# openai/tiktoken

Measured on AMD Instinct MI355X. Metric: GB/s text encoded (o200k_base-shaped vocab, 1 GiB corpus per GPU), bit-exact vs CoreBPE restatement, higher is better.
Workload: dtype u8; 1 GPU; o200k_shaped encode_ordinary_batch, 1024 MiB synthetic web-text per GPU (tkc_generate mix=1, seed 0x5EED0003), 318404 docs on rank 0, inputs resident in HBM, packed u32 output; encoding=o200k_shaped, pat_str_runs_on=hand-written scanners, bytes_per_gpu=1073741824, docs_rank0=318404, rccl_ranks=0, devices_visible=1, pieces_rank0=162498410, parallelism=doc-sharded x1

## Files before the change

tiktoken_amd/csrc/tk_common.h:

```cpp
#pragma once
#include <stdint.h>

#if defined(__HIPCC__)
#include <hip/hip_runtime.h>
#define TK_HD __host__ __device__ __forceinline__
#else
#define TK_HD inline
#endif

#define TK_RANK_MAX 0xFFFFFFFFu
#define TK_TILE 3840

enum : int {
    TK_DBG_SCANNERS = 4,
    TK_DBG_STARTS_ONLY = 8,
    TK_DBG_VERBOSE = 64,
    TK_DBG_KEEP_LONG = 0x80,
    TK_DBG_NO_MT = 256,
    TK_DBG_COLLIDE = 512,
    TK_DBG_ONE_MERGE = 1024,
    TK_DBG_NO_SMALL = 2048,
    TK_DBG_GENERIC = 0x100000,
    TK_DBG_NO_MID_CUT = 0x200000,
    TK_DBG_MERGE_PER_BIN = 0x800000,
    TK_DBG_NO_BUDGET = 0x20000000,
    TK_DBG_MAY_GIVE_UP = 0x8000000,
    TK_DBG_SECOND = 0x10000000,
    TK_DBG_HARD_ONLY = 0x40000000,
    TK_DBG_INTERNAL = TK_DBG_MAY_GIVE_UP | TK_DBG_SECOND | TK_DBG_HARD_ONLY,
};
constexpr int TK_DBG_USER[] = {TK_DBG_SCANNERS, TK_DBG_STARTS_ONLY, TK_DBG_VERBOSE, TK_DBG_KEEP_LONG, TK_DBG_NO_MT, TK_DBG_COLLIDE, TK_DBG_ONE_MERGE,
                               TK_DBG_NO_SMALL, TK_DBG_GENERIC, TK_DBG_NO_MID_CUT, TK_DBG_MERGE_PER_BIN, TK_DBG_NO_BUDGET};
constexpr bool tk_dbg_user_bits_disjoint() {
    int seen = TK_DBG_INTERNAL;
    for (int b : TK_DBG_USER) {
        if ((b & (b - 1)) != 0 || (seen & b) != 0) return false;
        seen |= b;
    }
    return true;
}
static_assert(tk_dbg_user_bits_disjoint(), "a debug bit a user sets is shared");

enum { TK_PAT_R50K = 0, TK_PAT_CL100K = 1, TK_PAT_O200K = 2 };

enum {
    TK_C_CONT = 0,
    TK_C_NL = 1,
    TK_C_SP = 2,
    TK_C_WSO = 3,
    TK_C_LU = 4,
    TK_C_LL = 5,
    TK_C_LC = 6,
    TK_C_MK = 7,
    TK_C_NU = 8,
    TK_C_AP = 9,
    TK_C_SL = 10,
    TK_C_OT = 11,
    TK_C_END = 12,
    TK_C_SPEC = 13,
};
#define TK_F_HARD 0x80u
#define TK_CB(c) (1u << (c))
#define TK_M_WS (TK_CB(TK_C_NL) | TK_CB(TK_C_SP) | TK_CB(TK_C_WSO))
#define TK_M_L (TK_CB(TK_C_LU) | TK_CB(TK_C_LL) | TK_CB(TK_C_LC))
#define TK_M_OTHER (TK_CB(TK_C_MK) | TK_CB(TK_C_AP) | TK_CB(TK_C_SL) | TK_CB(TK_C_OT))
#define TK_M_WORD (TK_M_L | TK_CB(TK_C_MK))
#define TK_M_UPPERISH (TK_CB(TK_C_LU) | TK_CB(TK_C_LC) | TK_CB(TK_C_MK))
#define TK_M_LOWERISH (TK_CB(TK_C_LL) | TK_CB(TK_C_LC) | TK_CB(TK_C_MK))

struct TkPieceSlot {
    uint64_t key;
    uint32_t rank;
    uint32_t len;
};
struct TkShortSlot {
    uint32_t key;
    uint32_t val;
};
#define TK_SHORT_EMPTY 0xFFFFFFFFu
#define TK_SHORT_RANK_MASK 0x3FFFFFFFu
#define TK_SHORT_MAX_RANK 0x3FFFFFFEu
#define TK_XL_MIN 9u
#define TK_XL_MAX 23u
struct alignas(16) TkXlSlot {
    uint64_t w0, w1, w2;
    uint32_t rank;
    uint32_t pad;
};
struct TkPairSlot {
    uint64_t key;
    uint32_t rank;
    uint32_t pad;
};
#define TK_EMPTY_KEY 0xFFFFFFFFFFFFFFFFull

struct TkPat {
    uint32_t w0;
    uint32_t c1;
    uint32_t c2[2];
    TK_HD constexpr int fam() const { return (int)(w0 & 3u); }
    TK_HD constexpr bool ci() const { return (w0 >> 2) & 1u; }
    TK_HD constexpr uint32_t suffix() const { return (w0 >> 3) & 3u; }
    TK_HD constexpr bool generic() const { return (w0 >> 5) & 1u; }
    TK_HD constexpr bool ws_dollar() const { return (w0 >> 6) & 1u; }
    TK_HD constexpr bool nl_rule() const { return (w0 >> 7) & 1u; }
    TK_HD constexpr uint32_t digits() const { return (w0 >> 8) & 0xFFu; }
    TK_HD constexpr uint32_t n2() const { return (w0 >> 16) & 7u; }
    TK_HD constexpr uint32_t two(uint32_t i) const { return (c2[i >> 1] >> (16u * (i & 1u))) & 0xFFFFu; }
    TK_HD constexpr uint32_t suffix_mask() const { return ((suffix() & 1u) ? TK_CB(TK_C_NL) : 0u) | ((suffix() & 2u) ? TK_CB(TK_C_SL) : 0u); }
    TK_HD constexpr bool same_as(const TkPat& o) const { return ((w0 ^ o.w0) & ~32u) == 0u && c1 == o.c1 && c2[0] == o.c2[0] && c2[1] == o.c2[1]; }
};
#define TK_PAT_GENERIC 3
TK_HD constexpr TkPat tk_stock_pat(int fam) {
    return TkPat{(uint32_t)fam | (fam != TK_PAT_R50K ? 4u : 0u) | (fam == TK_PAT_CL100K ? 8u : (fam == TK_PAT_O200K ? 24u : 0u)) |
                     (fam != TK_PAT_O200K ? 64u : 0u) | (fam != TK_PAT_R50K ? 128u : 0u) | (fam != TK_PAT_R50K ? (3u << 8) : 0u) | (3u << 16),
                 (1u << ('s' - 'a')) | (1u << ('t' - 'a')) | (1u << ('m' - 'a')) | (1u << ('d' - 'a')),
                 {((uint32_t)'l' << 8 | 'l') | (((uint32_t)'v' << 8 | 'e') << 16), ((uint32_t)'r' << 8 | 'e')}};
}

struct TkTables {
    const uint8_t* uc_stage1;
    const uint8_t* uc_stage2;
    const uint8_t* uc_bmp;
    const uint32_t* byte_tab;
    const TkShortSlot* short_tab;
    uint32_t short_mask, short_shift;
    const TkPieceSlot* mid_tab;
    uint32_t mid_mask, mid_shift;
    const TkPieceSlot* piece;
    const uint32_t* piece_off;
    uint64_t piece_mask;
    uint32_t max_token_len;
    const uint8_t* tok_bytes;
    const TkPairSlot* pair;
    const uint64_t* pair8;
    uint64_t pair_mask;
    const uint32_t* pair2;
    const uint32_t* byte_rank;
    const uint8_t* spec_bytes;
    const uint32_t* spec_off;
    const uint32_t* spec_id;
    const uint32_t* spec_head;
    uint32_t n_spec;
    uint32_t spec_first[8];
    uint32_t spec_fb;
    uint32_t n_spec_fb;
    uint32_t spec_second[8];
    int pattern;
    TkPat pat;
    uint16_t cert[16];
    const struct TkXlSlot* xl;
    uint32_t xl_mask;
    const uint32_t* xfilter;
};
#define TK_XFILTER_BITS (1u << 20)
TK_HD uint32_t tk_xfilter_bit(uint64_t ident_hash) { return (uint32_t)(ident_hash >> 32) & (TK_XFILTER_BITS - 1u); }

TK_HD uint64_t tk_mix64(uint64_t x) {
    x ^= x >> 32;
    x *= 0xD6E8FEB86659FD93ull;
    x ^= x >> 32;
    x *= 0xD6E8FEB86659FD93ull;
    x ^= x >> 32;
    return x;
}

TK_HD uint64_t tk_piece_slot_hash(uint64_t key, uint32_t len) {
    uint32_t x = (uint32_t)key * 0x9E3779B1u;
    x ^= x >> 15;
    x += (uint32_t)(key >> 32) * 0x85EBCA77u + len * 0xC2B2AE3Du;
    x ^= x >> 13;
    x *= 0x27D4EB2Fu;
    x ^= x >> 16;
    return x;
}
TK_HD uint32_t tk_short_slot(uint32_t key, uint32_t shift) { return (key * 0x9E3779B1u) >> shift; }
TK_HD uint32_t tk_mid_slot(uint64_t key, uint32_t shift) {
    uint32_t x = (uint32_t)key * 0x9E3779B1u + (uint32_t)(key >> 32) * 0x85EBCA77u;
    x ^= x >> 15;
    return (x * 0xC2B2AE3Du) >> shift;
}
TK_HD uint64_t tk_pair_slot_hash(uint64_t key) {
    uint32_t x = (uint32_t)key * 0x9E3779B1u + (uint32_t)(key >> 32) * 0x85EBCA77u;
    x ^= x >> 15;
    x *= 0x2C1B3C6Du;
    x ^= x >> 12;
    x *= 0x297A2D39u;
    x ^= x >> 15;
    return x;
}

TK_HD uint64_t tk_keep_bytes(uint64_t x, int r) {
    const uint32_t t4 = 4u * (8u - (uint32_t)(r < 0 ? 0 : (r > 8 ? 8 : r)));
    return (x << t4) << t4;
}
template <class Ld8>
TK_HD void tk_ident(Ld8&& ld8, uint32_t len, uint32_t where, uint64_t& w0, uint64_t& w1, uint64_t& w2) {
    const bool exact = len <= TK_XL_MAX;
    const uint64_t x0 = ld8(0u), x1 = ld8(exact ? 8u : len - 8u);
    w0 = tk_keep_bytes(x0, (int)len);
    w1 = exact ? tk_keep_bytes(x1, (int)len - 8) : x1;
    w2 = (1ull << 63) | ((uint64_t)len << 32) | where;
    if (exact) w2 = (tk_keep_bytes(ld8(16u), (int)len - 16) >> 8) | ((uint64_t)len << 56);
}
TK_HD uint64_t tk_ident_hash(uint64_t w0, uint64_t w1, uint64_t w2, bool exact) {
    const uint32_t a = (uint32_t)w0, b = (uint32_t)(w0 >> 32), c = (uint32_t)w1, d = (uint32_t)(w1 >> 32);
    const uint32_t e = exact ? (uint32_t)w2 : 0u, f = (uint32_t)(w2 >> 32);
    uint32_t h1 = a * 0x9E3779B1u + b * 0x85EBCA77u + c * 0xC2B2AE3Du + d * 0x27D4EB2Fu + e * 0x165667B1u + f * 0xD3A2646Du;
    h1 ^= h1 >> 15;
    h1 *= 0x2C1B3C6Du;
    h1 ^= h1 >> 12;
    uint32_t h2 = (a ^ 0x5BD1E995u) * 0x7FEB352Du + (b + d) * 0x846CA68Bu + (c ^ f) * 0xFD7046C5u + (e + ((a >> 19) | (a << 13))) * 0xB55A4F09u;
    h2 ^= h2 >> 13;
    h2 *= 0x9E3779B1u;
    h2 ^= h2 >> 16;
    return ((uint64_t)h2 << 32) | h1;
}

TK_HD uint64_t tk_hash_step(uint64_t h, uint64_t w) {
    uint64_t x = (h ^ w) * 0x9FB21C651E98DF25ull;
    x ^= x >> 29;
    return x + 0x9E3779B97F4A7C15ull;
}
#define TK_HASH_SEED 0x243F6A8885A308D3ull
#define TK_KEY_SAMPLED 32u
#define TK_PAIR8_ID_BITS 21
#define TK_PAIR8_MAX_ID ((1u << TK_PAIR8_ID_BITS) - 2u)
```

tiktoken_amd/csrc/tk_device.h:

```cpp
#pragma once
#include "tk_common.h"

TK_HD uint32_t tk_class_of_cp(const TkTables& T, uint32_t cp) {
    if (cp > 0x10FFFFu) return TK_C_OT;
    return T.uc_stage2[(uint32_t)T.uc_stage1[cp >> 8] * 256u + (cp & 255u)];
}

TK_HD uint32_t tk_classify_text(const TkTables& T, const uint8_t* __restrict__ text, uint64_t pos, uint64_t n) {
    uint32_t b = text[pos];
    if (b < 0x80u) return tk_class_of_cp(T, b);
    if ((b & 0xC0u) == 0x80u) return TK_C_CONT;
    uint32_t len = b >= 0xF0u ? 4u : (b >= 0xE0u ? 3u : 2u);
    if (pos + len > n) return TK_C_OT;
    uint32_t cp;
    if (len == 2u)
        cp = ((b & 0x1Fu) << 6) | (text[pos + 1] & 0x3Fu);
    else if (len == 3u)
        cp = ((b & 0x0Fu) << 12) | ((uint32_t)(text[pos + 1] & 0x3Fu) << 6) | (text[pos + 2] & 0x3Fu);
    else
        cp = ((b & 0x07u) << 18) | ((uint32_t)(text[pos + 1] & 0x3Fu) << 12) |
             ((uint32_t)(text[pos + 2] & 0x3Fu) << 6) | (text[pos + 3] & 0x3Fu);
    return tk_class_of_cp(T, cp);
}

// ... 480 lines not shown
            if (pat.generic() && !sx) break;
            sx &= sx - 1;
        }
        e = sx ? tk_ctz64(sx) : r;
        return e > TK_WIN_SAFE ? 0 : e;
    }
    uint32_t s = 0;
    bool s_ok = true;
    if (c == TK_C_SP && !nxt_end) s = k1;
    if (pat.fam() == TK_PAT_R50K) {
        int kind = -1;
        uint64_t b0 = 0;
        if ((w.get(TKB_L) >> s) & 1ull) { kind = TKB_L; b0 = w.get(TKB_L); }
        else if ((w.get(TKB_NU) >> s) & 1ull) { kind = TKB_NU; b0 = w.get(TKB_NU); }
        else if ((w.get(TKB_OTH) >> s) & 1ull) { kind = TKB_OTH; b0 = w.get(TKB_OTH); }
        if (kind >= 0) {
            uint32_t r = tk_runx(b0, stop, x, kind, s);
            return r == TK_UNRES ? 0 : s + r;
        }
        s_ok = false;
    } else if ((w.get(TKB_OTH) >> s) & 1ull) {
        uint32_t r = tk_runx(w.get(TKB_OTH), stop, x, TKB_OTH, s);
        if (r == TK_UNRES) return 0;
        const uint32_t e1 = s + r;
        uint32_t r2 = (pat.fam() == TK_PAT_O200K || pat.generic()) ? tk_runx(w.get(TKB_NLSL), stop, x, TKB_NLSL, e1) : tk_runx(w.get(TKB_NL), stop, x, TKB_NL, e1);
        return r2 == TK_UNRES ? 0 : e1 + r2;
    } else {
        s_ok = false;
    }
    (void)s_ok;
    {
        uint32_t q = tk_runx(w.get(TKB_WS), stop, x, TKB_WS, 0);
        if (q == TK_UNRES) return 0;
        if (q <= TK_WIN_SAFE) {
            uint64_t rng = tk_below(q);
            bool at_end = (stop >> q) & 1ull;
            uint64_t nlr = w.get(TKB_NL) & rng, st = w.start & rng;
            if (pat.ws_dollar() && at_end) return q;
            if (pat.nl_rule() && nlr) return 64u - tk_clz64(nlr);
            if (at_end) return q;
            if (tk_popc64(st) >= 2u) return 63u - tk_clz64(st);
            return q;
        }
        if (q + 1u > x.limit()) return 0;
        const bool at_end = tk_bitx(w.stop, x, TKB_HARD, q);
        if (pat.ws_dollar() && at_end) return q;
        if (pat.nl_rule()) {
            int ln = tk_last_setx(w.get(TKB_NL), x, TKB_NL, 0, q);
            if (ln >= 0) return (uint32_t)ln + 1u;
        }
        if (at_end) return q;
        return (uint32_t)tk_last_setx(w.start, x, TKB_START, 0, q);
    }
}

#define TK_WIN32_SAFE 26u
#if defined(__HIP_DEVICE_COMPILE__)
TK_HD uint32_t tk_w32_ctz(uint32_t v) { return v ? (uint32_t)(__ffs((int)v) - 1) : 32u; }
TK_HD uint32_t tk_w32_clz(uint32_t v) { return v ? (uint32_t)__clz((int)v) : 32u; }
TK_HD uint32_t tk_w32_popc(uint32_t v) { return (uint32_t)__popc(v); }
#else
TK_HD uint32_t tk_w32_ctz(uint32_t v) { return v ? (uint32_t)__builtin_ctz(v) : 32u; }
TK_HD uint32_t tk_w32_clz(uint32_t v) { return v ? (uint32_t)__builtin_clz(v) : 32u; }
TK_HD uint32_t tk_w32_popc(uint32_t v) { return (uint32_t)__builtin_popcount(v); }
#endif
TK_HD uint32_t tk_below32(uint32_t b) { return b >= 32u ? ~0u : ((1u << b) - 1u); }
TK_HD uint32_t tk_run32(uint32_t bits, uint32_t stop, uint32_t from) {
    return tk_w32_ctz(~((bits & ~stop) >> from));
}

template <class W32, class A>
TK_HD uint32_t tk_piece_len_bits32(const W32& w, A& a, uint64_t p, uint32_t c, TkPat pat) {
    const uint32_t stop = w.stop;
    const uint32_t k1 = 1u + tk_w32_ctz((w.start | stop) >> 1);
    if (k1 > 4u || c == TK_C_SPEC) return 0;
    const bool nxt_end = (stop >> k1) & 1u;
    uint32_t e = 0;
    if (pat.fam() == TK_PAT_O200K) {
        uint32_t ks = 64;
        if ((TK_M_WORD >> c) & 1u) ks = 0;
        else if (c != TK_C_NL && c != TK_C_NU && !nxt_end && (((w.get(TKB_UP) | w.get(TKB_LOW)) >> k1) & 1u)) ks = k1;
        if (ks != 64u) {
            const uint32_t re = ks + tk_run32(w.get(TKB_UP), stop, ks);
            if (re > TK_WIN32_SAFE) return 0;
            const uint32_t te = re + tk_run32(w.get(TKB_LOW), stop, re);
            if (te > TK_WIN32_SAFE) return 0;
            if (te > re) {
                e = te;
            } else {
                const uint32_t xx = w.get(TKB_CAS) & ~stop & tk_below32(re) & ~tk_below32(ks);
                e = xx ? 32u - tk_w32_clz(xx) : re;
            }
            if (!((stop >> e) & 1u) && a.byte(p + e) == '\'') e += tk_contraction_bits(w, a, p, e, pat);
            return e;
        }
    } else if (pat.fam() == TK_PAT_CL100K) {
        if (c == TK_C_AP) {
            const uint32_t k = tk_contraction_bits(w, a, p, 0, pat);
            if (k) return k;
        }
        if ((TK_M_L >> c) & 1u) {
            const uint32_t r = tk_run32(w.get(TKB_L), stop, 0);
            return r > TK_WIN32_SAFE ? 0 : r;
        }
        if (c != TK_C_NL && c != TK_C_NU && !nxt_end && ((w.get(TKB_L) >> k1) & 1u)) {
            const uint32_t r = k1 + tk_run32(w.get(TKB_L), stop, k1);
            return r > TK_WIN32_SAFE ? 0 : r;
        }
    } else {
        if (c == TK_C_AP) {
            const uint32_t k = tk_contraction_bits(w, a, p, 0, pat);
            if (k) return k;
        }
    }
    if (pat.fam() != TK_PAT_R50K && c == TK_C_NU) {
        const uint32_t r = tk_run32(w.get(TKB_NU), stop, 0);
        uint32_t sx = pat.digits() ? (w.start & tk_below32(r)) : 0u;
        for (uint32_t i = 0; i < pat.digits(); ++i) {
            if (pat.generic() && !sx) break;
            sx &= sx - 1;
        }
        e = sx ? tk_w32_ctz(sx) : r;
        return e > TK_WIN32_SAFE ? 0 : e;
    }
    uint32_t s = 0;
    if (c == TK_C_SP && !nxt_end) s = k1;
    if (pat.fam() == TK_PAT_R50K) {
        int kind = -1;
        if ((w.get(TKB_L) >> s) & 1u) kind = TKB_L;
        else if ((w.get(TKB_NU) >> s) & 1u) kind = TKB_NU;
        else if ((w.get(TKB_OTH) >> s) & 1u) kind = TKB_OTH;
        if (kind >= 0) {
            const uint32_t r = s + tk_run32(w.get(kind), stop, s);
            return r > TK_WIN32_SAFE ? 0 : r;
        }
    } else if ((w.get(TKB_OTH) >> s) & 1u) {
        const uint32_t e1 = s + tk_run32(w.get(TKB_OTH), stop, s);
        if (e1 > TK_WIN32_SAFE) return 0;
        const uint32_t e2 = e1 + tk_run32((pat.fam() == TK_PAT_O200K || pat.generic()) ? w.get(TKB_NLSL) : w.get(TKB_NL), stop, e1);
        return e2 > TK_WIN32_SAFE ? 0 : e2;
    }
    const uint32_t q = tk_run32(w.get(TKB_WS), stop, 0);
    if (q > TK_WIN32_SAFE) return 0;
    const uint32_t rng = tk_below32(q);
    const bool at_end = (stop >> q) & 1u;
    const uint32_t nlr = w.get(TKB_NL) & rng, st = w.start & rng;
    if (pat.ws_dollar() && at_end) return q;
    if (pat.nl_rule() && nlr) return 32u - tk_w32_clz(nlr);
    if (at_end) return q;
    if (tk_w32_popc(st) >= 2u) return 31u - tk_w32_clz(st);
    return q;
}

TK_HD uint32_t tk_probe_short_from(const TkTables& T, uint32_t key, uint32_t len, uint32_t i, TkShortSlot s) {
    for (;;) {
        if (s.key == key && (s.val >> 30) == len - 1u && s.val != TK_SHORT_EMPTY) return s.val & TK_SHORT_RANK_MASK;
        if (s.val == TK_SHORT_EMPTY) return TK_RANK_MAX;
        i = (i + 1u) & T.short_mask;
        s = T.short_tab[i];
    }
}
TK_HD uint32_t tk_probe_short(const TkTables& T, uint32_t key, uint32_t len) {
    const uint32_t i = tk_short_slot(key, T.short_shift);
    return tk_probe_short_from(T, key, len, i, T.short_tab[i]);
}
TK_HD uint32_t tk_probe_mid_from(const TkTables& T, uint64_t key, uint32_t len, uint32_t i, TkPieceSlot s) {
    for (;;) {
        if (s.key == key && s.len == len) return s.rank;
        if (s.len == 0u) return TK_RANK_MAX;
        i = (i + 1u) & T.mid_mask;
        s = T.mid_tab[i];
    }
}
TK_HD uint32_t tk_probe_mid(const TkTables& T, uint64_t key, uint32_t len) {
    const uint32_t i = tk_mid_slot(key, T.mid_shift);
    return tk_probe_mid_from(T, key, len, i, T.mid_tab[i]);
}
template <class Verify>
TK_HD uint32_t tk_probe_piece_from(const TkTables& T, uint64_t key, uint32_t len, uint64_t i, TkPieceSlot s, Verify verify) {
    for (;;) {
        if (s.key == TK_EMPTY_KEY && s.len == 0u) return TK_RANK_MAX;
        if (s.key == key && s.len == len && verify(T.piece_off[i])) return s.rank;
        i = (i + 1) & T.piece_mask;
        s = T.piece[i];
    }
}
template <class Verify>
TK_HD uint32_t tk_probe_piece(const TkTables& T, uint64_t key, uint32_t len, Verify verify) {
    const uint64_t i = tk_piece_slot_hash(key, len) & T.piece_mask;
    return tk_probe_piece_from(T, key, len, i, T.piece[i], verify);
}

TK_HD uint32_t tk_probe_xl_from(const TkTables& T, uint64_t w0, uint64_t w1, uint64_t w2, uint32_t i, TkXlSlot s) {
    for (;;) {
        if (s.rank == TK_RANK_MAX) return TK_RANK_MAX;
        if (s.w0 == w0 && s.w1 == w1 && s.w2 == w2) return s.rank;
        i = (i + 1u) & T.xl_mask;
        s = T.xl[i];
    }
}
TK_HD uint32_t tk_probe_xl(const TkTables& T, uint64_t w0, uint64_t w1, uint64_t w2) {
    const uint32_t i = (uint32_t)tk_ident_hash(w0, w1, w2, true) & T.xl_mask;
    return tk_probe_xl_from(T, w0, w1, w2, i, T.xl[i]);
}

TK_HD uint32_t tk_probe_pair(const TkTables& T, uint32_t a, uint32_t b) {
    if (T.pair8) {
        const uint64_t key = ((uint64_t)a << TK_PAIR8_ID_BITS) | b;
        uint64_t bk = tk_pair_slot_hash(key) & T.pair_mask;
        for (;;) {
            const uint64_t* p = T.pair8 + bk * 4;
#if defined(__HIP_DEVICE_COMPILE__)
            const ulonglong2 v0 = *(const ulonglong2*)p, v1 = *(const ulonglong2*)(p + 2);
            const uint64_t s0 = v0.x, s1 = v0.y, s2 = v1.x, s3 = v1.y;
#else
            const uint64_t s0 = p[0], s1 = p[1], s2 = p[2], s3 = p[3];
#endif
            if ((s0 >> 22) == key) return (uint32_t)(s0 & 0x3FFFFFu);
            if ((s1 >> 22) == key) return (uint32_t)(s1 & 0x3FFFFFu);
            if ((s2 >> 22) == key) return (uint32_t)(s2 & 0x3FFFFFu);
            if ((s3 >> 22) == key) return (uint32_t)(s3 & 0x3FFFFFu);
            if (s3 == TK_EMPTY_KEY) return TK_RANK_MAX;
            bk = (bk + 1) & T.pair_mask;
        }
    }
    uint64_t key = ((uint64_t)a << 32) | b;
    uint64_t i = tk_pair_slot_hash(key) & T.pair_mask;
    for (;;) {
        TkPairSlot s = T.pair[i];
        if (s.key == key) return s.rank;
        if (s.key == TK_EMPTY_KEY) return TK_RANK_MAX;
        i = (i + 1) & T.pair_mask;
    }
}

TK_HD uint64_t tk_load8(const uint8_t* __restrict__ text, uint64_t pos) {
    uintptr_t a = (uintptr_t)(text + pos);
    const uint64_t* w = (const uint64_t*)(a & ~(uintptr_t)7);
    uint32_t sh = (uint32_t)(a & 7u) * 8u;
    uint64_t lo = w[0];
    if (sh == 0) return lo;
    uint64_t hi = w[1];
    return (lo >> sh) | (hi << (64u - sh));
}

TK_HD uint64_t tk_mask_low_bytes(uint64_t w, uint32_t nbytes) {
    return nbytes >= 8u ? w : (w & ((1ull << (nbytes * 8u)) - 1ull));
}

TK_HD uint64_t tk_key_of_text(const uint8_t* __restrict__ text, uint64_t pos, uint32_t len) {
    if (len <= 8u) return tk_mask_low_bytes(tk_load8(text, pos), len);
    if (len > TK_KEY_SAMPLED) {
        uint64_t h = TK_HASH_SEED ^ ((uint64_t)len << 32);
        h = tk_hash_step(h, tk_load8(text, pos));
        h = tk_hash_step(h, tk_load8(text, pos + 8u));
        h = tk_hash_step(h, tk_load8(text, pos + len - 16u));
        h = tk_hash_step(h, tk_load8(text, pos + len - 8u));
        return h == TK_EMPTY_KEY ? 0 : h;
    }
    uint64_t h = TK_HASH_SEED;
    uint32_t i = 0;
    for (; i + 8u <= len; i += 8u) h = tk_hash_step(h, tk_load8(text, pos + i));
    if (i < len) h = tk_hash_step(h, tk_mask_low_bytes(tk_load8(text, pos + i), len - i));
    if (h == TK_EMPTY_KEY) h = 0;
    return h;
}

TK_HD bool tk_equal_bytes(const uint8_t* text, uint64_t pos, const uint8_t* blob, uint32_t off, uint32_t len) {
    uint32_t i = 0;
    for (; i + 8u <= len; i += 8u)
        if (tk_load8(text, pos + i) != tk_load8(blob, (uint64_t)off + i)) return false;
    if (i < len) {
        uint32_t r = len - i;
        if (tk_mask_low_bytes(tk_load8(text, pos + i), r) != tk_mask_low_bytes(tk_load8(blob, (uint64_t)off + i), r)) return false;
    }
    return true;
}

TK_HD uint32_t tk_lookup_text_piece(const TkTables& T, const uint8_t* __restrict__ text, uint64_t pos, uint32_t len) {
    if (len <= 8u) {
        const uint64_t key = tk_mask_low_bytes(tk_load8(text, pos), len);
        if (len <= 4u && T.short_tab) return tk_probe_short(T, (uint32_t)key, len);
        return tk_probe_mid(T, key, len);
    }
    if (len > T.max_token_len) return TK_RANK_MAX;
    uint64_t key = tk_key_of_text(text, pos, len);
    return tk_probe_piece(T, key, len, [&](uint32_t off) { return tk_equal_bytes(text, pos, T.tok_bytes, off, len); });
}

#if defined(__HIP_DEVICE_COMPILE__)
TK_HD int tk_ffs32(uint32_t v) { return __ffs((int)v); }
TK_HD int tk_clz32(uint32_t v) { return __clz((int)v); }
TK_HD int tk_popc32(uint32_t v) { return __popc(v); }
#else
TK_HD int tk_ffs32(uint32_t v) { return __builtin_ffs((int)v); }
TK_HD int tk_clz32(uint32_t v) { return v ? __builtin_clz(v) : 32; }
TK_HD int tk_popc32(uint32_t v) { return __builtin_popcount(v); }
#endif

struct TkMask128 {
    uint64_t lo, hi;
    TK_HD void clear(uint32_t k) {
        if (k < 64u) lo &= ~(1ull << k);
        else hi &= ~(1ull << (k - 64u));
    }
    TK_HD bool test(uint32_t k) const { return k < 64u ? (lo >> k) & 1ull : (hi >> (k - 64u)) & 1ull; }
    TK_HD uint32_t next_after(uint32_t k) const {
        if (k < 63u) {
            uint64_t l = lo & ~((2ull << k) - 1ull);
            if (l) return tk_ctz64(l);
        }
        uint64_t h = hi;
        if (k >= 127u) h = 0;
        else if (k >= 64u) h &= ~((2ull << (k - 64u)) - 1ull);
        if (h) return 64u + tk_ctz64(h);
        return 128u;
    }
    TK_HD int prev_before(uint32_t k) const {
        uint64_t h = k > 64u ? hi & ((1ull << (k - 64u)) - 1ull) : 0ull;
        if (h) return 127 - (int)tk_clz64(h);
        uint64_t l = k >= 64u ? lo : lo & ((1ull << k) - 1ull);
        if (l) return 63 - (int)tk_clz64(l);
        return -1;
    }
};

template <int STRIDE>
TK_HD uint32_t tk_lane_merge(const TkTables& T, const uint8_t* __restrict__ text, uint64_t s, uint32_t n, uint32_t* id, uint32_t* rk,
                             uint32_t* __restrict__ out) {
    uint32_t pb = text[s];
    for (uint32_t k = 0; k < n; ++k) {
        uint32_t nb = k + 1 < n ? text[s + k + 1] : 0u;
        id[k * STRIDE] = T.byte_rank[pb];
        rk[k * STRIDE] = k + 1 < n ? T.pair2[(pb << 8) | nb] : TK_RANK_MAX;
        pb = nb;
    }
    TkMask128 alive;
    alive.lo = n >= 64u ? ~0ull : ((1ull << n) - 1ull);
    alive.hi = n > 64u ? (n >= 128u ? ~0ull : ((1ull << (n - 64u)) - 1ull)) : 0ull;
    for (;;) {
        uint32_t best = TK_RANK_MAX, bi = 0;
        for (uint32_t k = 0; k + 1 < n; ++k) {
            uint32_t r = rk[k * STRIDE];
            if (r < best) {
                best = r;
                bi = k;
            }
        }
        if (best == TK_RANK_MAX) break;
        const uint32_t j = alive.next_after(bi);
        alive.clear(j);
        id[bi * STRIDE] = best;
        rk[j * STRIDE] = TK_RANK_MAX;
        const uint32_t nn = alive.next_after(bi);
        const int pp = alive.prev_before(bi);
        uint32_t r_i = TK_RANK_MAX, r_p = TK_RANK_MAX;
// ... 11 lines not shown
```

tiktoken_amd/csrc/tk_tables.cpp:

```cpp
#include "tk_tables.h"

#include <stdio.h>
#include <stdlib.h>
#include <string.h>

#include <algorithm>
#include <array>
#include <chrono>
#include <numeric>
#include <thread>

int tk_pattern_id(const char* pat_str) {
    TkPat p;
    TkRxCompiled rx;
    if (!tk_compile_pattern(pat_str, &p, nullptr, &rx).empty()) return -1;
    return rx.empty() ? p.fam() : 3;
}

TkPat tk_nosplit_pat() { return TkPat{(uint32_t)TK_PAT_R50K | 32u, 0u, {0u, 0u}}; }

std::string tk_compile_pattern(const char* pat_str, TkPat* pat, uint16_t* cert, TkRxCompiled* rx) {
    const char* dbg = getenv("TIKTOKEN_AMD_DEBUG");
    const bool force_generic = dbg && (atoi(dbg) & TK_DBG_GENERIC);
    const std::string perr = force_generic ? std::string("generic engine forced by TIKTOKEN_AMD_DEBUG") : tk_parse_pattern(pat_str, pat, cert);
    if (perr.empty()) return "";
    const std::string rerr = tk_rx_compile(pat_str, rx);
    if (!rerr.empty()) {
        rx->ins.clear();
        return "pat_str is not supported: " + rerr + " [and it is not one of the hand-written scanner families: " + perr + "]";
    }
    *pat = tk_nosplit_pat();
    if (cert) memset(cert, 0, 16 * sizeof(uint16_t));
    return "";
}

uint64_t tk_key_of_bytes(const uint8_t* p, uint32_t len) {
    if (len <= 8) {
        uint64_t k = 0;
        memcpy(&k, p, len);
        return k;
    }
    if (len > TK_KEY_SAMPLED) {
        uint64_t h = TK_HASH_SEED ^ ((uint64_t)len << 32);
        for (uint32_t o : {0u, 8u, len - 16u, len - 8u}) {
            uint64_t w;
            memcpy(&w, p + o, 8);
            h = tk_hash_step(h, w);
        }
        return h == TK_EMPTY_KEY ? 0 : h;
    }
    uint64_t h = TK_HASH_SEED;
    uint32_t i = 0;
    for (; i + 8 <= len; i += 8) {
        uint64_t w;
        memcpy(&w, p + i, 8);
        h = tk_hash_step(h, w);
    }
    if (i < len) {
        uint64_t w = 0;
        memcpy(&w, p + i, len - i);
        h = tk_hash_step(h, w);
    }
    if (h == TK_EMPTY_KEY) h = 0;
    return h;
}

uint32_t TkHostTables::lookup_piece(const uint8_t* p, uint32_t len) const {
    if (len == 0) return TK_RANK_MAX;
    if (len <= 8) {
        uint64_t key = 0;
        memcpy(&key, p, len);
        if (len <= 4 && !short_tab.empty()) {
            uint32_t i = tk_short_slot((uint32_t)key, short_shift);
            for (;;) {
                const TkShortSlot& s = short_tab[i];
                if (s.val == TK_SHORT_EMPTY) return TK_RANK_MAX;
                if (s.key == (uint32_t)key && (s.val >> 30) == len - 1) return s.val & TK_SHORT_RANK_MASK;
                i = (i + 1) & short_mask;
            }
        }
        if (mid_tab.empty()) return TK_RANK_MAX;
        uint32_t i = tk_mid_slot(key, mid_shift);
        for (;;) {
            const TkPieceSlot& s = mid_tab[i];
            if (s.len == 0) return TK_RANK_MAX;
            if (s.key == key && s.len == len) return s.rank;
            i = (i + 1) & mid_mask;
        }
    }
    if (piece.empty()) return TK_RANK_MAX;
    uint64_t key = tk_key_of_bytes(p, len);
    uint64_t i = tk_piece_slot_hash(key, len) & piece_mask;
    for (;;) {
        const TkPieceSlot& s = piece[i];
        if (s.key == TK_EMPTY_KEY && s.len == 0) return TK_RANK_MAX;
        if (s.key == key && s.len == len) {
            if (memcmp(tok_bytes.data() + piece_off[i], p, len) == 0) return s.rank;
        }
        i = (i + 1) & piece_mask;
    }
}

uint32_t TkHostTables::lookup_pair(uint32_t a, uint32_t b) const {
    if (!pair8.empty()) {
        const uint64_t key = ((uint64_t)a << TK_PAIR8_ID_BITS) | b;
        uint64_t bk = tk_pair_slot_hash(key) & pair_mask;
        for (;;) {
            for (int j = 0; j < 4; ++j) {
                uint64_t s = pair8[bk * 4 + j];
                if ((s >> 22) == key) return (uint32_t)(s & 0x3FFFFFu);
                if (s == TK_EMPTY_KEY) return TK_RANK_MAX;
            }
            bk = (bk + 1) & pair_mask;
        }
    }
    uint64_t key = ((uint64_t)a << 32) | b;
    uint64_t i = tk_pair_slot_hash(key) & pair_mask;
    for (;;) {
        const TkPairSlot& s = pair[i];
        if (s.key == TK_EMPTY_KEY) return TK_RANK_MAX;
        if (s.key == key) return s.rank;
        i = (i + 1) & pair_mask;
    }
}

std::string tk_build_tables(const uint8_t* ranks_blob, const uint64_t* ranks_off, const uint32_t* ranks_ids,
                            uint64_t n_ranks, const uint8_t* spec_blob, const uint64_t* spec_off,
                            const uint32_t* spec_ids, uint64_t n_spec, const char* pat_str, TkHostTables* out) {
    TkHostTables& T = *out;
    const bool timing = getenv("TIKTOKEN_AMD_TIMING") != nullptr;
    auto t_prev = std::chrono::steady_clock::now();
    auto lap = [&](const char* what) {
        const auto now = std::chrono::steady_clock::now();
        if (timing) fprintf(stderr, "tk_build_tables: %-28s %7.1f ms\n", what, std::chrono::duration<double, std::milli>(now - t_prev).count());
        t_prev = now;
    };
    {
        const std::string perr = tk_compile_pattern(pat_str, &T.pat, T.cert, &T.rx);
        if (!perr.empty()) return perr;
        T.pattern = T.pat.fam();
    }
    lap("pattern");
    if (n_ranks == 0) return "mergeable_ranks is empty";
    if (ranks_off[n_ranks] >= 0xFFFFFFFFull) return "vocabulary byte blob too large";
    T.n_ranks = n_ranks;
    T.tok_bytes.assign(ranks_blob, ranks_blob + ranks_off[n_ranks]);
    T.tok_bytes.resize(T.tok_bytes.size() + 16, 0);

    uint32_t max_rank = 0;
    uint64_t n_short = 0, n_mid = 0, n_long = 0, n_xl = 0;
    for (uint64_t k = 0; k < n_ranks; ++k) {
        max_rank = std::max(max_rank, ranks_ids[k] == TK_RANK_MAX ? 0u : ranks_ids[k]);
        const uint64_t len = ranks_off[k + 1] - ranks_off[k];
        (len <= 4 ? n_short : (len <= 8 ? n_mid : n_long)) += 1;
        if (len >= TK_XL_MIN && len <= TK_XL_MAX) ++n_xl;
    }
    for (uint64_t k = 0; k < n_spec; ++k) max_rank = std::max(max_rank, spec_ids[k]);
    if (max_rank >= 0x7FFFFFFFu)
        return "token ids of 2^31 - 1 and above are not supported (the per-piece result word keeps its top bit for pieces that are not a "
               "single token, and one value for text that yields no token)";
    const bool use_short = max_rank <= TK_SHORT_MAX_RANK;
    if (!use_short) {
        n_mid += n_short;
        n_short = 0;
    }
    auto pow2_for = [](uint64_t items, uint32_t* mask, uint32_t* shift) {
        uint32_t bits = 6;
        while ((1ull << bits) < 2 * items + 2) ++bits;
        *mask = (uint32_t)((1ull << bits) - 1);
        *shift = 32 - bits;
        return (uint64_t)1 << bits;
    };
    if (use_short) T.short_tab.assign(pow2_for(n_short, &T.short_mask, &T.short_shift), TkShortSlot{0xFFFFFFFFu, TK_SHORT_EMPTY});
    T.mid_tab.assign(pow2_for(n_mid, &T.mid_mask, &T.mid_shift), TkPieceSlot{TK_EMPTY_KEY, TK_RANK_MAX, 0});
    uint64_t cap = 64;
    while (cap < 2 * n_long + 2) cap <<= 1;
    T.piece_mask = cap - 1;
    T.piece.assign(cap, TkPieceSlot{TK_EMPTY_KEY, TK_RANK_MAX, 0});
    T.piece_off.assign(cap, 0);
    {
        uint64_t xcap = 64;
        while (2 * xcap < 5 * n_xl + 2) xcap <<= 1;
        T.xl_mask = (uint32_t)(xcap - 1);
        T.xl.assign(xcap, TkXlSlot{~0ull, ~0ull, ~0ull, TK_RANK_MAX, 0u});
        T.xfilter.assign(TK_XFILTER_BITS / 32, 0u);
    }
    for (int b = 0; b < 256; ++b) T.byte_rank[b] = TK_RANK_MAX;
    T.pair2.assign(65536, TK_RANK_MAX);
    {
        uint32_t mr = 0;
        for (uint64_t k = 0; k < n_ranks; ++k) mr = std::max(mr, ranks_ids[k] == TK_RANK_MAX ? 0u : ranks_ids[k]);
        T.max_rank = mr;
        T.dec_is_dense = (uint64_t)mr < 4 * n_ranks + 65536;
        if (T.dec_is_dense) T.dec_dense.assign((size_t)mr + 1, std::make_pair(0u, 0u));
        else T.dec_sparse.reserve(n_ranks * 2);
    }
    uint64_t pr_short = 0, pr_mid = 0, pr_long = 0, pr_xl = 0;
    for (uint64_t k = 0; k < n_ranks; ++k) {
        uint64_t o = ranks_off[k], len64 = ranks_off[k + 1] - o;
        if (len64 == 0) return "mergeable_ranks contains an empty key";
        uint32_t len = (uint32_t)len64, rank = ranks_ids[k];
        if (rank == TK_RANK_MAX) return "rank 0xFFFFFFFF is reserved (Rank::MAX sentinel, src/lib.rs:53)";
        const uint8_t* p = ranks_blob + o;
        if (T.lookup_piece(p, len) != TK_RANK_MAX) return "duplicate key in mergeable_ranks";
        bool fresh;
        if (T.dec_is_dense) {
            fresh = T.dec_dense[rank].second == 0;
            T.dec_dense[rank] = std::make_pair((uint32_t)o, len);
        } else {
            fresh = T.dec_sparse.emplace(rank, std::make_pair((uint32_t)o, len)).second;
        }
        if (!fresh)
            return "Encoder and decoder must be of equal length. Maybe you had duplicate token indices in your "
                   "encoder?";
        if (len <= 8) {
            uint64_t key = 0;
            memcpy(&key, p, len);
            if (len <= 4 && use_short) {
                uint32_t i = tk_short_slot((uint32_t)key, T.short_shift);
                ++pr_short;
                while (T.short_tab[i].val != TK_SHORT_EMPTY) {
                    i = (i + 1) & T.short_mask;
                    ++pr_short;
                }
                T.short_tab[i] = TkShortSlot{(uint32_t)key, rank | ((len - 1) << 30)};
            } else {
                uint32_t i = tk_mid_slot(key, T.mid_shift);
                ++pr_mid;
                while (T.mid_tab[i].len != 0) {
                    i = (i + 1) & T.mid_mask;
                    ++pr_mid;
                }
                T.mid_tab[i] = TkPieceSlot{key, rank, len};
            }
        } else {
            uint64_t key = tk_key_of_bytes(p, len);
            uint64_t i = tk_piece_slot_hash(key, len) & T.piece_mask;
            ++pr_long;
            while (!(T.piece[i].key == TK_EMPTY_KEY && T.piece[i].len == 0)) {
                i = (i + 1) & T.piece_mask;
                ++pr_long;
            }
            T.piece[i] = TkPieceSlot{key, rank, len};
            T.piece_off[i] = (uint32_t)o;
            uint64_t w0, w1, w2;
            tk_ident([&](uint32_t at) {
                uint64_t w = 0;
                memcpy(&w, p + at, at < len ? std::min<uint32_t>(8u, len - at) : 0u);
                return w;
            }, len, 0u, w0, w1, w2);
            if (len > TK_XL_MAX) {
                uint64_t hh = tk_ident_hash(w0, w1, w2, false);
                if (hh == TK_EMPTY_KEY) hh = 0;
                const uint32_t bit = tk_xfilter_bit(hh);
                T.xfilter[bit >> 5] |= 1u << (bit & 31u);
            }
            if (len >= TK_XL_MIN && len <= TK_XL_MAX) {
                uint32_t j = (uint32_t)tk_ident_hash(w0, w1, w2, true) & T.xl_mask;
                ++pr_xl;
                while (T.xl[j].rank != TK_RANK_MAX) {
                    j = (j + 1) & T.xl_mask;
                    ++pr_xl;
                }
                T.xl[j] = TkXlSlot{w0, w1, w2, rank, 0u};
            }
        }
        if (len == 1) T.byte_rank[p[0]] = rank;
        if (len == 2) T.pair2[((uint32_t)p[0] << 8) | p[1]] = rank;
        if (len > T.max_token_len) T.max_token_len = len;
    }
    T.probes_short = n_short ? (double)pr_short / (double)n_short : 0;
    T.probes_mid = n_mid ? (double)pr_mid / (double)n_mid : 0;
    T.probes_long = n_long ? (double)pr_long / (double)n_long : 0;
    T.probes_xl = n_xl ? (double)pr_xl / (double)n_xl : 0;
    for (int b = 0; b < 256; ++b)
        if (T.byte_rank[b] == TK_RANK_MAX)
            return "every single byte must be a key of mergeable_ranks (byte_pair_encode indexes ranks[piece] for "
                   "1-byte pieces, src/lib.rs:201-203)";

    lap("piece tables + decoder");
    std::vector<TkPairSlot> entries;
    {
        unsigned nth = std::thread::hardware_concurrency();
        nth = nth == 0 ? 1 : (nth > 32 ? 32 : nth);
        if (const char* e = getenv("TIKTOKEN_AMD_BUILD_THREADS")) nth = (unsigned)std::max(1, atoi(e));
        if (n_ranks < 4096) nth = 1;
        const uint64_t nblocks = (n_ranks + 255) / 256;
        std::vector<std::vector<TkPairSlot>> part(nblocks);
        auto work = [&](unsigned t) {
            for (uint64_t b = t; b < nblocks; b += nth) {
                std::vector<TkPairSlot>& e = part[b];
                for (uint64_t k = b * 256; k < b * 256 + 256 && k < n_ranks; ++k) {
                    uint64_t o = ranks_off[k];
                    uint32_t len = (uint32_t)(ranks_off[k + 1] - o), rank = ranks_ids[k];
                    const uint8_t* p = ranks_blob + o;
                    for (uint32_t s = 1; s < len; ++s) {
                        uint32_t a = T.lookup_piece(p, s);
                        if (a == TK_RANK_MAX) continue;
                        uint32_t b2 = T.lookup_piece(p + s, len - s);
                        if (b2 == TK_RANK_MAX) continue;
                        e.push_back(TkPairSlot{((uint64_t)a << 32) | b2, rank, 0});
                    }
                }
            }
        };
        std::vector<std::thread> th;
        for (unsigned t = 1; t < nth; ++t) th.emplace_back(work, t);
        work(0);
        for (auto& x : th) x.join();
        size_t tot = 0;
        for (auto& e : part) tot += e.size();
        entries.reserve(tot);
        for (auto& e : part) entries.insert(entries.end(), e.begin(), e.end());
    }
    T.n_pairs = entries.size();
    lap("pair entries");

    uint32_t max_id = 0;
    for (uint64_t k = 0; k < n_ranks; ++k) max_id = std::max(max_id, ranks_ids[k]);
    if (max_id <= TK_PAIR8_MAX_ID) {
        uint64_t nb = 16;
        while ((double)nb * 4 * 0.5 < (double)entries.size() + 1) nb <<= 1;
        T.pair_mask = nb - 1;
        T.pair8.assign(nb * 4, TK_EMPTY_KEY);
        for (const TkPairSlot& e : entries) {
            const uint64_t key = ((e.key >> 32) << TK_PAIR8_ID_BITS) | (e.key & 0xFFFFFFFFull);
            uint64_t bk = tk_pair_slot_hash(key) & T.pair_mask;
            for (;;) {
                int j = 0;
                while (j < 4 && T.pair8[bk * 4 + j] != TK_EMPTY_KEY) ++j;
                if (j < 4) {
                    T.pair8[bk * 4 + j] = (key << 22) | e.rank;
                    break;
                }
                bk = (bk + 1) & T.pair_mask;
            }
        }
    } else {
        cap = 64;
        while ((double)cap * 0.4 < (double)entries.size() + 1) cap <<= 1;
        T.pair_mask = cap - 1;
        T.pair.assign(cap, TkPairSlot{TK_EMPTY_KEY, TK_RANK_MAX, 0});
        for (const TkPairSlot& e : entries) {
            uint64_t i = tk_pair_slot_hash(e.key) & T.pair_mask;
            while (T.pair[i].key != TK_EMPTY_KEY) i = (i + 1) & T.pair_mask;
            T.pair[i] = e;
        }
    }

    lap("pair table");
    std::vector<uint64_t> order(n_spec);
    std::iota(order.begin(), order.end(), 0);
    auto sbytes = [&](uint64_t k) { return std::string((const char*)spec_blob + spec_off[k], spec_off[k + 1] - spec_off[k]); };
    std::sort(order.begin(), order.end(), [&](uint64_t a, uint64_t b) { return sbytes(a) < sbytes(b); });
    memset(T.spec_first, 0, sizeof T.spec_first);
    T.spec_off.push_back(0);
    for (uint64_t idx : order) {
        std::string s = sbytes(idx);
        if (s.empty()) return "empty special token";
        T.spec_decoder.emplace(spec_ids[idx], std::make_pair((uint32_t)T.spec_bytes.size(), (uint32_t)s.size()));
        T.spec_bytes.insert(T.spec_bytes.end(), s.begin(), s.end());
        T.spec_off.push_back((uint32_t)T.spec_bytes.size());
        T.spec_id.push_back(spec_ids[idx]);
        unsigned char f = (unsigned char)s[0];
        T.spec_first[f >> 5] |= 1u << (f & 31);
    }
    for (size_t i = 1; i < order.size(); ++i)
        if (sbytes(order[i]) == sbytes(order[i - 1])) return "duplicate special token string";
    T.spec_bytes.resize(T.spec_bytes.size() + 16, 0);

    lap("special tokens");
    return "";
}

const std::vector<uint32_t>& TkHostTables::sorted_ranks() const {
    std::call_once(sorted_once_, [this] {
        struct E {
            uint32_t rank, off, len;
        };
        std::vector<E> v;
        v.reserve(n_ranks);
        for_each_token([&](uint32_t r, uint32_t o, uint32_t l) { v.push_back(E{r, o, l}); });
        const uint8_t* b = tok_bytes.data();
        std::sort(v.begin(), v.end(), [b](const E& x, const E& y) {
            const int c = memcmp(b + x.off, b + y.off, x.len < y.len ? x.len : y.len);
            return c < 0 || (c == 0 && x.len < y.len);
        });
        sorted_ranks_.resize(v.size());
        for (size_t i = 0; i < v.size(); ++i) sorted_ranks_[i] = v[i].rank;
    });
    return sorted_ranks_;
}


std::string tk_parse_tiktoken(const uint8_t* text, uint64_t len, std::vector<uint8_t>* blob, std::vector<uint64_t>* off,
                              std::vector<uint32_t>* ids) {
    static const std::array<int8_t, 256> dec = [] {
        std::array<int8_t, 256> d;
        d.fill(-1);
        const char* al = "ABCDEFGHIJKLMNOPQRSTUVWXYZabcdefghijklmnopqrstuvwxyz0123456789+/";
        for (int i = 0; i < 64; ++i) d[(unsigned char)al[i]] = (int8_t)i;
        return d;
    }();
    auto is_ws = [](uint8_t c) { return c == ' ' || (c >= 9 && c <= 13); };
    blob->clear();
    off->assign(1, 0);
    ids->clear();
    blob->reserve(len / 2);
    uint64_t line_no = 0, i = 0;
    auto bad = [&](const char* what) { return std::string("Error parsing line ") + std::to_string(line_no) + " of the .tiktoken data: " + what; };
    while (i < len) {
        ++line_no;
        uint64_t e = i;
        while (e < len && text[e] != '\n' && text[e] != '\r') ++e;
        const uint64_t a0 = i, b0 = e;
        i = e + 1;
// ... 59 lines not shown
```

Measured before the change: 176.1 GB/s.

## Switch short, mid and identity token tables to bucketed probing with wide loads

Replaces the per-slot linear probing in the short (≤4 byte), mid (≤8 byte) and by-identity token hash tables with fixed-width buckets of 4, 2 and 2 slots. On the device each bucket is fetched with 16-byte vector loads. A 'passed' marker on the last slot of an overflowed bucket lets a miss stop after one bucket instead of walking to an empty slot. Table construction now places keys bucket-wise, sets the overflow markers, and rejects vocabularies that need more than 64 consecutive full buckets. The aim is fewer dependent memory round trips per piece lookup during encoding. The cost is more bytes read per probe and a new build-time failure mode.

Result: faster. 181.6 GB/s, median of 6 (+3.2%).

```diff
diff --git a/tiktoken_amd/csrc/tk_common.h b/tiktoken_amd/csrc/tk_common.h
--- a/tiktoken_amd/csrc/tk_common.h
+++ b/tiktoken_amd/csrc/tk_common.h
@@ -73,6 +73,7 @@
     uint32_t rank;
     uint32_t len;
 };
+#define TK_MID_PASSED 0x100u
 struct TkShortSlot {
     uint32_t key;
     uint32_t val;
@@ -85,7 +86,7 @@
 struct alignas(16) TkXlSlot {
     uint64_t w0, w1, w2;
     uint32_t rank;
-    uint32_t pad;
+    uint32_t passed;
 };
 struct TkPairSlot {
     uint64_t key;
@@ -217,6 +218,73 @@
     return ((uint64_t)h2 << 32) | h1;
 }
 
+#define TK_SHORT_BW 4u
+#define TK_MID_BW 2u
+#define TK_XL_BW 2u
+#define TK_BUCKET_BOUND 64u
+
+TK_HD uint32_t tk_bucket_probe_short(const TkShortSlot* tab, uint32_t mask, uint32_t slot, uint32_t key, uint32_t len) {
+    const uint32_t tag = (len - 1u) << 30;
+    for (uint32_t b = slot & ~(TK_SHORT_BW - 1u);; b = (b + TK_SHORT_BW) & mask) {
+        const TkShortSlot* p = tab + b;
+#if defined(__HIP_DEVICE_COMPILE__)
+        const uint4 q0 = *(const uint4*)p, q1 = *(const uint4*)(p + 2);
+        const uint32_t k0 = q0.x, v0 = q0.y, k1 = q0.z, v1 = q0.w, k2 = q1.x, v2 = q1.y, k3 = q1.z, v3 = q1.w;
+#else
+        const uint32_t k0 = p[0].key, v0 = p[0].val, k1 = p[1].key, v1 = p[1].val, k2 = p[2].key, v2 = p[2].val, k3 = p[3].key, v3 = p[3].val;
+#endif
+        uint32_t v = TK_SHORT_EMPTY;
+        if (k3 == key && ((v3 ^ tag) >> 30) == 0u) v = v3;
+        if (k2 == key && ((v2 ^ tag) >> 30) == 0u) v = v2;
+        if (k1 == key && ((v1 ^ tag) >> 30) == 0u) v = v1;
+        if (k0 == key && ((v0 ^ tag) >> 30) == 0u) v = v0;
+        if (v != TK_SHORT_EMPTY) return v & TK_SHORT_RANK_MASK;
+        if (v3 == TK_SHORT_EMPTY) return TK_RANK_MAX;
+    }
+}
+TK_HD uint32_t tk_bucket_probe_mid(const TkPieceSlot* tab, uint32_t mask, uint32_t slot, uint64_t key, uint32_t len) {
+    for (uint32_t b = slot & ~(TK_MID_BW - 1u);; b = (b + TK_MID_BW) & mask) {
+        const TkPieceSlot* p = tab + b;
+#if defined(__HIP_DEVICE_COMPILE__)
+        const uint4 q0 = *(const uint4*)p, q1 = *(const uint4*)(p + 1);
+        const uint64_t k0 = ((uint64_t)q0.y << 32) | q0.x, k1 = ((uint64_t)q1.y << 32) | q1.x;
+        const uint32_t r0 = q0.z, l0 = q0.w, r1 = q1.z, l1 = q1.w;
+#else
+        const uint64_t k0 = p[0].key, k1 = p[1].key;
+        const uint32_t r0 = p[0].rank, l0 = p[0].len, r1 = p[1].rank, l1 = p[1].len;
+#endif
+        if (k0 == key && l0 == len) return r0;
+        if (k1 == key && (l1 & 0xFFu) == len) return r1;
+        if (l1 < TK_MID_PASSED) return TK_RANK_MAX;
+    }
+}
+TK_HD uint32_t tk_bucket_probe_xl(const TkXlSlot* tab, uint32_t mask, uint32_t slot, uint64_t w0, uint64_t w1, uint64_t w2) {
+    for (uint32_t b = slot & ~(TK_XL_BW - 1u);; b = (b + TK_XL_BW) & mask) {
+        const TkXlSlot* p = tab + b;
+#if defined(__HIP_DEVICE_COMPILE__)
+        const ulonglong2 a0 = *(const ulonglong2*)p, a1 = *((const ulonglong2*)p + 1), c0 = *((const ulonglong2*)p + 2), c1 = *((const ulonglong2*)p + 3);
+        const uint64_t x0 = a0.x, x1 = a0.y, x2 = a1.x, y0 = c0.x, y1 = c0.y, y2 = c1.x;
+        const uint32_t r0 = (uint32_t)a1.y, r1 = (uint32_t)c1.y, passed = (uint32_t)(c1.y >> 32);
+#else
+        const uint64_t x0 = p[0].w0, x1 = p[0].w1, x2 = p[0].w2, y0 = p[1].w0, y1 = p[1].w1, y2 = p[1].w2;
+        const uint32_t r0 = p[0].rank, r1 = p[1].rank, passed = p[1].passed;
+#endif
+        if (x0 == w0 && x1 == w1 && x2 == w2) return r0;
+        if (y0 == w0 && y1 == w1 && y2 == w2) return r1;
+        if (!passed) return TK_RANK_MAX;
+    }
+}
+template <class Full, class Pass>
+inline uint32_t tk_bucket_place(uint32_t bw, uint32_t mask, uint32_t slot, Full&& full, Pass&& pass) {
+    uint32_t b = slot & ~(bw - 1u);
+    for (uint32_t step = 0; step < TK_BUCKET_BOUND; ++step, b = (b + bw) & mask) {
+        for (uint32_t j = 0; j < bw; ++j)
+            if (!full(b + j)) return b + j;
+        pass(b + bw - 1u);
+    }
+    return 0xFFFFFFFFu;
+}
+
 TK_HD uint64_t tk_hash_step(uint64_t h, uint64_t w) {
     uint64_t x = (h ^ w) * 0x9FB21C651E98DF25ull;
     x ^= x >> 29;
diff --git a/tiktoken_amd/csrc/tk_device.h b/tiktoken_amd/csrc/tk_device.h
--- a/tiktoken_amd/csrc/tk_device.h
+++ b/tiktoken_amd/csrc/tk_device.h
@@ -656,29 +656,11 @@
     return q;
 }
 
-TK_HD uint32_t tk_probe_short_from(const TkTables& T, uint32_t key, uint32_t len, uint32_t i, TkShortSlot s) {
-    for (;;) {
-        if (s.key == key && (s.val >> 30) == len - 1u && s.val != TK_SHORT_EMPTY) return s.val & TK_SHORT_RANK_MASK;
-        if (s.val == TK_SHORT_EMPTY) return TK_RANK_MAX;
-        i = (i + 1u) & T.short_mask;
-        s = T.short_tab[i];
-    }
-}
 TK_HD uint32_t tk_probe_short(const TkTables& T, uint32_t key, uint32_t len) {
-    const uint32_t i = tk_short_slot(key, T.short_shift);
-    return tk_probe_short_from(T, key, len, i, T.short_tab[i]);
-}
-TK_HD uint32_t tk_probe_mid_from(const TkTables& T, uint64_t key, uint32_t len, uint32_t i, TkPieceSlot s) {
-    for (;;) {
-        if (s.key == key && s.len == len) return s.rank;
-        if (s.len == 0u) return TK_RANK_MAX;
-        i = (i + 1u) & T.mid_mask;
-        s = T.mid_tab[i];
-    }
+    return tk_bucket_probe_short(T.short_tab, T.short_mask, tk_short_slot(key, T.short_shift), key, len);
 }
 TK_HD uint32_t tk_probe_mid(const TkTables& T, uint64_t key, uint32_t len) {
-    const uint32_t i = tk_mid_slot(key, T.mid_shift);
-    return tk_probe_mid_from(T, key, len, i, T.mid_tab[i]);
+    return tk_bucket_probe_mid(T.mid_tab, T.mid_mask, tk_mid_slot(key, T.mid_shift), key, len);
 }
 template <class Verify>
 TK_HD uint32_t tk_probe_piece_from(const TkTables& T, uint64_t key, uint32_t len, uint64_t i, TkPieceSlot s, Verify verify) {
@@ -695,17 +677,8 @@
     return tk_probe_piece_from(T, key, len, i, T.piece[i], verify);
 }
 
-TK_HD uint32_t tk_probe_xl_from(const TkTables& T, uint64_t w0, uint64_t w1, uint64_t w2, uint32_t i, TkXlSlot s) {
-    for (;;) {
-        if (s.rank == TK_RANK_MAX) return TK_RANK_MAX;
-        if (s.w0 == w0 && s.w1 == w1 && s.w2 == w2) return s.rank;
-        i = (i + 1u) & T.xl_mask;
-        s = T.xl[i];
-    }
-}
 TK_HD uint32_t tk_probe_xl(const TkTables& T, uint64_t w0, uint64_t w1, uint64_t w2) {
-    const uint32_t i = (uint32_t)tk_ident_hash(w0, w1, w2, true) & T.xl_mask;
-    return tk_probe_xl_from(T, w0, w1, w2, i, T.xl[i]);
+    return tk_bucket_probe_xl(T.xl, T.xl_mask, (uint32_t)tk_ident_hash(w0, w1, w2, true) & T.xl_mask, w0, w1, w2);
 }
 
 TK_HD uint32_t tk_probe_pair(const TkTables& T, uint32_t a, uint32_t b) {
diff --git a/tiktoken_amd/csrc/tk_tables.cpp b/tiktoken_amd/csrc/tk_tables.cpp
--- a/tiktoken_amd/csrc/tk_tables.cpp
+++ b/tiktoken_amd/csrc/tk_tables.cpp
@@ -70,23 +70,9 @@
     if (len <= 8) {
         uint64_t key = 0;
         memcpy(&key, p, len);
-        if (len <= 4 && !short_tab.empty()) {
-            uint32_t i = tk_short_slot((uint32_t)key, short_shift);
-            for (;;) {
-                const TkShortSlot& s = short_tab[i];
-                if (s.val == TK_SHORT_EMPTY) return TK_RANK_MAX;
-                if (s.key == (uint32_t)key && (s.val >> 30) == len - 1) return s.val & TK_SHORT_RANK_MASK;
-                i = (i + 1) & short_mask;
-            }
-        }
+        if (len <= 4 && !short_tab.empty()) return tk_bucket_probe_short(short_tab.data(), short_mask, tk_short_slot((uint32_t)key, short_shift), (uint32_t)key, len);
         if (mid_tab.empty()) return TK_RANK_MAX;
-        uint32_t i = tk_mid_slot(key, mid_shift);
-        for (;;) {
-            const TkPieceSlot& s = mid_tab[i];
-            if (s.len == 0) return TK_RANK_MAX;
-            if (s.key == key && s.len == len) return s.rank;
-            i = (i + 1) & mid_mask;
-        }
+        return tk_bucket_probe_mid(mid_tab.data(), mid_mask, tk_mid_slot(key, mid_shift), key, len);
     }
     if (piece.empty()) return TK_RANK_MAX;
     uint64_t key = tk_key_of_bytes(p, len);
@@ -196,6 +182,11 @@
         else T.dec_sparse.reserve(n_ranks * 2);
     }
     uint64_t pr_short = 0, pr_mid = 0, pr_long = 0, pr_xl = 0;
+    auto too_deep = [](const char* which) {
+        return std::string("the ") + which + " token table cannot take this vocabulary: more than " + std::to_string(TK_BUCKET_BOUND) +
+               " full buckets in a row (token bytes chosen to collide?)";
+    };
+    auto bucket_steps = [](uint32_t slot, uint32_t home, uint32_t bw, uint32_t mask) { return (((slot & ~(bw - 1u)) - (home & ~(bw - 1u))) & mask) / bw + 1u; };
     for (uint64_t k = 0; k < n_ranks; ++k) {
         uint64_t o = ranks_off[k], len64 = ranks_off[k + 1] - o;
         if (len64 == 0) return "mergeable_ranks contains an empty key";
@@ -217,20 +208,16 @@
             uint64_t key = 0;
             memcpy(&key, p, len);
             if (len <= 4 && use_short) {
-                uint32_t i = tk_short_slot((uint32_t)key, T.short_shift);
-                ++pr_short;
-                while (T.short_tab[i].val != TK_SHORT_EMPTY) {
-                    i = (i + 1) & T.short_mask;
-                    ++pr_short;
-                }
+                const uint32_t h = tk_short_slot((uint32_t)key, T.short_shift);
+                const uint32_t i = tk_bucket_place(TK_SHORT_BW, T.short_mask, h, [&](uint32_t j) { return T.short_tab[j].val != TK_SHORT_EMPTY; }, [](uint32_t) {});
+                if (i == 0xFFFFFFFFu) return too_deep("short");
+                pr_short += bucket_steps(i, h, TK_SHORT_BW, T.short_mask);
                 T.short_tab[i] = TkShortSlot{(uint32_t)key, rank | ((len - 1) << 30)};
             } else {
-                uint32_t i = tk_mid_slot(key, T.mid_shift);
-                ++pr_mid;
-                while (T.mid_tab[i].len != 0) {
-                    i = (i + 1) & T.mid_mask;
-                    ++pr_mid;
-                }
+                const uint32_t h = tk_mid_slot(key, T.mid_shift);
+                const uint32_t i = tk_bucket_place(TK_MID_BW, T.mid_mask, h, [&](uint32_t j) { return T.mid_tab[j].len != 0; }, [&](uint32_t j) { T.mid_tab[j].len |= TK_MID_PASSED; });
+                if (i == 0xFFFFFFFFu) return too_deep("mid");
+                pr_mid += bucket_steps(i, h, TK_MID_BW, T.mid_mask);
                 T.mid_tab[i] = TkPieceSlot{key, rank, len};
             }
         } else {
@@ -256,12 +243,10 @@
                 T.xfilter[bit >> 5] |= 1u << (bit & 31u);
             }
             if (len >= TK_XL_MIN && len <= TK_XL_MAX) {
-                uint32_t j = (uint32_t)tk_ident_hash(w0, w1, w2, true) & T.xl_mask;
-                ++pr_xl;
-                while (T.xl[j].rank != TK_RANK_MAX) {
-                    j = (j + 1) & T.xl_mask;
-                    ++pr_xl;
-                }
+                const uint32_t h = (uint32_t)tk_ident_hash(w0, w1, w2, true) & T.xl_mask;
+                const uint32_t j = tk_bucket_place(TK_XL_BW, T.xl_mask, h, [&](uint32_t q) { return T.xl[q].rank != TK_RANK_MAX; }, [&](uint32_t q) { T.xl[q].passed = 1u; });
+                if (j == 0xFFFFFFFFu) return too_deep("by-identity");
+                pr_xl += bucket_steps(j, h, TK_XL_BW, T.xl_mask);
                 T.xl[j] = TkXlSlot{w0, w1, w2, rank, 0u};
             }
         }
```
